# scroll-tech/zkevm-circuits

Measured on NVIDIA H100. Metric: SuperCircuit-shaped k=20 create_proof seconds (halo2 KZG/SHPLONK, Blake2b transcript), lower is better.
Workload: dtype u256 (8x u32 Montgomery limbs, BN254 Fr/Fq)

## Files before the change

### zkevm-circuits_b200/csrc/expr.cu

```cuda
#include <type_traits>
#include "common.cuh"
#include "expr.cuh"

namespace zkb {

struct ExprLaunch {
    const Instr *code;
    uint32_t ncode;
    const Fr *const *cols;
    const Fr *consts;
    Fr *const *outs;
    uint32_t log_n;
    uint32_t out_stride;
    uint32_t out_offset;
};

template <int NREGS, int THREADS, bool SMEM>
struct RegFile {
    uint4 *lo, *hi;
    Fr loc[SMEM ? 1 : NREGS];
    __device__ __forceinline__ RegFile(uint4 *base) : lo(base + threadIdx.x), hi(base + NREGS * THREADS + threadIdx.x) {}
    __device__ __forceinline__ Fr get(uint32_t r) const {
        if (!SMEM) return loc[r];
        const uint4 a = lo[r * THREADS], b = hi[r * THREADS];
        Fr v;
        v.l[0] = a.x; v.l[1] = a.y; v.l[2] = a.z; v.l[3] = a.w;
        v.l[4] = b.x; v.l[5] = b.y; v.l[6] = b.z; v.l[7] = b.w;
        return v;
    }
    __device__ __forceinline__ void set(uint32_t r, const Fr &v) {
        if (!SMEM) { loc[r] = v; return; }
        lo[r * THREADS] = make_uint4(v.l[0], v.l[1], v.l[2], v.l[3]);
        hi[r * THREADS] = make_uint4(v.l[4], v.l[5], v.l[6], v.l[7]);
    }
};

struct FlagLaunch {
    const Instr *code;
    uint32_t ncode;
    const Fr *const *cols;
    const Fr *consts;
    uint32_t *bits;
    uint32_t words;
    uint32_t log_n;
};

template <int NREGS, int THREADS, bool SMEM, class Launch>
__device__ __forceinline__ void run_program(const Launch &L, uint32_t tid) {
    constexpr bool FLAG = std::is_same<Launch, FlagLaunch>::value;
    extern __shared__ uint4 expr_smem[];
    const uint32_t mask = (1u << L.log_n) - 1, row = tid & mask;
    RegFile<NREGS, THREADS, SMEM> regs(expr_smem);
    Fr acc = Fr::zero(), acc2 = Fr::zero();
    uint32_t pc = 0;
    auto col = [&](uint32_t imm) {
        const int32_t rot = (int32_t)(int16_t)(imm >> 16);
        return fp_load(L.cols[imm & 0xffffu] + ((row + (uint32_t)rot) & mask));
    };
    auto cst = [&](uint32_t i) { return fp_load(L.consts + i); };
    auto arg = [&]() { return L.code[++pc].imm; };
    for (; pc < L.ncode; ++pc) {
        const Instr in = L.code[pc];
        Fr x, y;
        switch (in.op) {
        case OP_LOADCOL: regs.set(in.dst, col(in.imm)); continue;
        case OP_LOADCONST: regs.set(in.dst, cst(in.imm)); continue;
        case OP_ADD: x = regs.get(in.a); y = regs.get(in.b); goto add;
        case OP_ADD_RC + FORM_RC: x = regs.get(in.a); y = col(in.imm); goto add;
        case OP_ADD_RC + FORM_CR: x = col(in.imm); y = regs.get(in.a); goto add;
        case OP_ADD_RC + FORM_RK: x = regs.get(in.a); y = cst(in.imm); goto add;
        case OP_ADD_RC + FORM_KR: x = cst(in.imm); y = regs.get(in.a); goto add;
        case OP_ADD_RC + FORM_CC: x = col(in.imm); y = col(arg()); goto add;
        case OP_ADD_RC + FORM_CK: x = col(in.imm); y = cst(arg()); goto add;
        case OP_ADD_RC + FORM_KC: x = cst(in.imm); y = col(arg()); goto add;
        case OP_SUB: x = regs.get(in.a); y = regs.get(in.b); goto sub;
        case OP_SUB_RC + FORM_RC: x = regs.get(in.a); y = col(in.imm); goto sub;
        case OP_SUB_RC + FORM_CR: x = col(in.imm); y = regs.get(in.a); goto sub;
        case OP_SUB_RC + FORM_RK: x = regs.get(in.a); y = cst(in.imm); goto sub;
        case OP_SUB_RC + FORM_KR: x = cst(in.imm); y = regs.get(in.a); goto sub;
        case OP_SUB_RC + FORM_CC: x = col(in.imm); y = col(arg()); goto sub;
        case OP_SUB_RC + FORM_CK: x = col(in.imm); y = cst(arg()); goto sub;
        case OP_SUB_RC + FORM_KC: x = cst(in.imm); y = col(arg()); goto sub;
        case OP_MUL: x = regs.get(in.a); y = regs.get(in.b); goto mul;
        case OP_MUL_RC + FORM_RC: x = regs.get(in.a); y = col(in.imm); goto mul;
        case OP_MUL_RC + FORM_CR: x = col(in.imm); y = regs.get(in.a); goto mul;
        case OP_MUL_RC + FORM_RK: x = regs.get(in.a); y = cst(in.imm); goto mul;
        case OP_MUL_RC + FORM_KR: x = cst(in.imm); y = regs.get(in.a); goto mul;
        case OP_MUL_RC + FORM_CC: x = col(in.imm); y = col(arg()); goto mul;
        case OP_MUL_RC + FORM_CK: x = col(in.imm); y = cst(arg()); goto mul;
        case OP_MUL_RC + FORM_KC: x = cst(in.imm); y = col(arg()); goto mul;
        case OP_NEG: regs.set(in.dst, fp_neg(regs.get(in.a))); continue;
        case OP_FLAG:
            if constexpr (FLAG) {
                const uint32_t b = __ballot_sync(0xffffffffu, tid < (1u << L.log_n) && !regs.get(in.a).is_zero());
                const uint32_t word = tid >> 5;
                if ((threadIdx.x & 31) == 0 && word < L.words) L.bits[(size_t)in.imm * L.words + word] = b;
            }
            continue;
        case OP_HORNER: case OP_HORNER_C:
            if constexpr (!FLAG) acc = fp_add(fp_mul(acc, cst(in.imm)), in.op == OP_HORNER ? regs.get(in.a) : col(arg()));
            continue;
        case OP_HORNER2: case OP_HORNER2_C:
            if constexpr (!FLAG) acc2 = fp_add(fp_mul(acc2, cst(in.imm)), in.op == OP_HORNER2 ? regs.get(in.a) : col(arg()));
            continue;
        case OP_FOLD: case OP_FOLD_C:
            if constexpr (!FLAG) {
                acc = fp_add(fp_mul(acc, cst(in.imm)), fp_mul(in.op == OP_FOLD ? regs.get(in.a) : col(arg()), acc2));
                acc2 = Fr::zero();
            }
            continue;
        case OP_STORE:
            if constexpr (!FLAG) fp_store(L.outs[in.imm] + (size_t)row * L.out_stride + L.out_offset, regs.get(in.a));
            continue;
        case OP_STOREACC:
            if constexpr (!FLAG) fp_store(L.outs[in.imm & 0xffu] + (size_t)row * L.out_stride + L.out_offset, fp_mul(acc, cst(in.imm >> 8)));
            continue;
        case OP_CLEARACC: acc = Fr::zero(); continue;
        default: continue;
        }
    add: regs.set(in.dst, fp_add(x, y)); continue;
    sub: regs.set(in.dst, fp_sub(x, y)); continue;
    mul: regs.set(in.dst, fp_mul(x, y));
    }
}

template <int NREGS, int THREADS, bool SMEM>
__global__ void __launch_bounds__(THREADS) expr_kernel(ExprLaunch L) {
    const uint32_t row = blockIdx.x * blockDim.x + threadIdx.x;
    if (row >= (1u << L.log_n)) return;
    run_program<NREGS, THREADS, SMEM>(L, row);
}

template <int NREGS, int THREADS, bool SMEM>
__global__ void __launch_bounds__(THREADS) expr_flag_kernel(FlagLaunch L) {
    run_program<NREGS, THREADS, SMEM>(L, blockIdx.x * blockDim.x + threadIdx.x);
}

template <class Launch, int NREGS, int THREADS, void (*KERNEL)(Launch)>
static int32_t launch_smem(const Launch &L, uint32_t n, cudaStream_t st) {
    constexpr size_t bytes = (size_t)NREGS * THREADS * 32;
    static bool attr_set[64] = {};
    int dev = 0;
    cudaGetDevice(&dev);
    if (bytes > 48 * 1024 && dev < 64 && !attr_set[dev]) {
        ZKB_CUDA(cudaFuncSetAttribute(KERNEL, cudaFuncAttributeMaxDynamicSharedMemorySize, (int)bytes));
        attr_set[dev] = true;
    }
    KERNEL<<<(n + THREADS - 1) / THREADS, THREADS, bytes, st>>>(L);
    return ZKB_OK;
}

int32_t expr_run_device(zkb_ctx *ctx, const Instr *d_code, uint32_t ncode, int nregs, const Fr *const *d_cols, const Fr *d_consts,
                        Fr *const *d_outs, uint32_t log_n, uint32_t out_stride, uint32_t out_offset, cudaStream_t st) {
    ExprLaunch L{d_code, ncode, d_cols, d_consts, d_outs, log_n, out_stride, out_offset};
    const uint32_t n = 1u << log_n;
    const unsigned blocks = (n + 127) / 128;
    ProfScope ps_(ctx, PROF_EXPR, st);
    if (nregs <= 8) ZKB_TRY((launch_smem<ExprLaunch, 8, 128, expr_kernel<8, 128, true>>(L, n, st)));
    else if (nregs <= 16) ZKB_TRY((launch_smem<ExprLaunch, 16, 128, expr_kernel<16, 128, true>>(L, n, st)));
    else expr_kernel<64, 128, false><<<blocks, 128, 0, st>>>(L);
    ctx->launches++;
    ZKB_CUDA(cudaGetLastError());
    return ZKB_OK;
}

int32_t expr_flag_run_device(zkb_ctx *ctx, const Instr *d_code, uint32_t ncode, int nregs, const Fr *const *d_cols, const Fr *d_consts,
                             uint32_t *bits, uint32_t words, uint32_t log_n, cudaStream_t st) {
    FlagLaunch L{d_code, ncode, d_cols, d_consts, bits, words, log_n};
    const uint32_t n = 1u << log_n;
    if (nregs <= 8) ZKB_TRY((launch_smem<FlagLaunch, 8, 128, expr_flag_kernel<8, 128, true>>(L, n, st)));
    else if (nregs <= 16) ZKB_TRY((launch_smem<FlagLaunch, 16, 128, expr_flag_kernel<16, 128, true>>(L, n, st)));
    else expr_flag_kernel<64, 128, false><<<(n + 127) / 128, 128, 0, st>>>(L);
    ctx->launches++;
    ZKB_CUDA(cudaGetLastError());
    return ZKB_OK;
}

}
```

### zkevm-circuits_b200/csrc/expr.cuh

```cuda
#pragma once
#include <stdint.h>
#include <algorithm>
#include <array>
#include <map>
#include <string>
#include <tuple>
#include <vector>
#include "ff.cuh"

namespace zkb {

enum : uint8_t {
    OP_LOADCOL = 0,
    OP_LOADCONST = 1,
    OP_ADD = 2,
    OP_SUB = 3,
    OP_MUL = 4,
    OP_NEG = 5,
    OP_HORNER = 6,
    OP_STORE = 7,
    OP_STOREACC = 8,
    OP_CLEARACC = 9,
    OP_HORNER2 = 10,
    OP_FOLD = 11,
    OP_FLAG = 12,
    OP_ARG = 13,
    FORM_RC = 0, FORM_CR = 1, FORM_RK = 2, FORM_KR = 3, FORM_CC = 4, FORM_CK = 5, FORM_KC = 6,
    OP_ADD_RC = 16,
    OP_SUB_RC = 24,
    OP_MUL_RC = 32,
    OP_HORNER_C = 40,
    OP_HORNER2_C = 41,
    OP_FOLD_C = 42,
};

struct alignas(8) Instr {
    uint8_t op, dst, a, b;
    uint32_t imm;
};

constexpr int EXPR_MAX_REGS = 64;

struct ENode {
    uint8_t kind;
    uint32_t a, b;
};

class ExprBuilder {
public:
    std::vector<ENode> nodes;
    std::vector<Fr> consts;
    std::vector<uint32_t> degree;

    uint32_t col(uint32_t slot, int32_t rot) { return intern(0, slot, (uint32_t)rot); }
    uint32_t constant(const Fr &v) {
        std::array<uint32_t, 8> key;
        for (int i = 0; i < 8; ++i) key[i] = v.l[i];
        auto it = const_index.find(key);
        uint32_t idx;
        if (it == const_index.end()) {
            idx = (uint32_t)consts.size();
            consts.push_back(v);
            const_index.emplace(key, idx);
        } else idx = it->second;
        return intern(1, idx, 0);
    }
    uint32_t add(uint32_t x, uint32_t y) { return intern(2, x, y); }
    uint32_t sub(uint32_t x, uint32_t y) { return intern(3, x, y); }
    uint32_t mul(uint32_t x, uint32_t y) { return intern(4, x, y); }
    uint32_t neg(uint32_t x) { return intern(5, x, 0); }
    uint32_t const_slot(const Fr &v) {
        uint32_t n = constant(v);
        return nodes[n].a;
    }
    void columns(uint32_t root, std::vector<char> &seen, std::vector<char> &used) const {
        std::vector<uint32_t> stack{root};
        while (!stack.empty()) {
            const uint32_t v = stack.back();
            stack.pop_back();
            if (seen[v]) continue;
            seen[v] = 1;
            const ENode &e = nodes[v];
            if (e.kind == 0) used[e.a] = 1;
            else if (e.kind >= 2) {
                stack.push_back(e.a);
                if (e.kind != 5) stack.push_back(e.b);
            }
        }
    }

private:
    std::map<std::tuple<uint8_t, uint32_t, uint32_t>, uint32_t> index;
    std::map<std::array<uint32_t, 8>, uint32_t> const_index;
    uint32_t intern(uint8_t kind, uint32_t a, uint32_t b) {
        auto key = std::make_tuple(kind, a, b);
        auto it = index.find(key);
        if (it != index.end()) return it->second;
        nodes.push_back(ENode{kind, a, b});
        degree.push_back(kind == 0 ? 1 : kind == 1 ? 0 : kind == 4 ? degree[a] + degree[b] : kind == 5 ? degree[a] : std::max(degree[a], degree[b]));
        index.emplace(key, (uint32_t)nodes.size() - 1);
        return (uint32_t)nodes.size() - 1;
    }
};

class ProgramBuilder {
public:
    explicit ProgramBuilder(ExprBuilder &eb) : eb(eb) {}
    std::vector<Instr> code;
    int max_regs_used = 0;
    std::string error;

    enum RootAction { HORNER, STORE, HORNER2, FOLD, FLAG };
    struct Root { uint32_t node; RootAction action; uint32_t imm; };
    bool scope(const std::vector<Root> &roots);
    void clear_acc() { code.push_back(Instr{OP_CLEARACC, 0, 0, 0, 0}); }
    void store_acc(uint32_t out_slot, uint32_t scale_const_index) {
        code.push_back(Instr{OP_STOREACC, 0, 0, 0, out_slot | (scale_const_index << 8)});
    }

private:
    ExprBuilder &eb;
    void fuse(size_t begin);
};

inline void ProgramBuilder::fuse(size_t begin) {
    auto is_arith = [](uint8_t op) { return op == OP_ADD || op == OP_SUB || op == OP_MUL; };
    auto is_root = [](uint8_t op) { return op == OP_HORNER || op == OP_HORNER2 || op == OP_FOLD; };
    auto is_load = [](uint8_t op) { return op == OP_LOADCOL || op == OP_LOADCONST; };
    auto reads = [&](const Instr &in, int s) {
        if (is_arith(in.op)) return true;
        return s == 0 && (in.op == OP_NEG || is_root(in.op) || in.op == OP_STORE || in.op == OP_FLAG);
    };
    auto writes = [&](const Instr &in) { return is_load(in.op) || is_arith(in.op) || in.op == OP_NEG; };
    const size_t end = code.size();
    std::vector<std::array<int64_t, 2>> src(end - begin, {-1, -1});
    for (size_t i = begin; i < end; ++i) {
        if (!is_load(code[i].op)) continue;
        const uint8_t r = code[i].dst;
        int uses = 0, slot = -1;
        size_t user = 0;
        for (size_t j = i + 1; j < end && uses < 2; ++j) {
            for (int s = 0; s < 2; ++s)
                if (reads(code[j], s) && (s == 0 ? code[j].a : code[j].b) == r) { ++uses; user = j; slot = s; }
            if (writes(code[j]) && code[j].dst == r) break;
        }
        if (uses != 1) continue;
        const uint8_t op = code[user].op;
        if (is_arith(op) || (is_root(op) && code[i].op == OP_LOADCOL)) src[user - begin][slot] = (int64_t)i;
    }
    auto kind = [&](const std::array<int64_t, 2> &s, int k) { return s[k] < 0 ? 'R' : code[s[k]].op == OP_LOADCOL ? 'C' : 'K'; };
    std::vector<bool> fused(end - begin, false);
    for (auto &s : src) {
        if (kind(s, 0) == 'K' && kind(s, 1) == 'K') s[1] = -1;
        for (int k = 0; k < 2; ++k)
            if (s[k] >= 0) fused[s[k] - begin] = true;
    }
    std::vector<Instr> out;
    for (size_t i = begin; i < end; ++i) {
        const Instr in = code[i];
        const auto &s = src[i - begin];
        if (fused[i - begin]) continue;
        if (s[0] < 0 && s[1] < 0) { out.push_back(in); continue; }
        if (is_root(in.op)) {
            const uint8_t op = in.op == OP_HORNER ? OP_HORNER_C : in.op == OP_HORNER2 ? OP_HORNER2_C : OP_FOLD_C;
            out.push_back(Instr{op, 0, 0, 0, in.imm});
            out.push_back(Instr{OP_ARG, 0, 0, 0, code[s[0]].imm});
            continue;
        }
        const char ka = kind(s, 0), kb = kind(s, 1);
        const int form = ka == 'R' ? (kb == 'C' ? FORM_RC : FORM_RK)
                       : kb == 'R' ? (ka == 'C' ? FORM_CR : FORM_KR)
                       : ka == 'C' ? (kb == 'C' ? FORM_CC : FORM_CK) : FORM_KC;
        const uint8_t base = in.op == OP_ADD ? OP_ADD_RC : in.op == OP_SUB ? OP_SUB_RC : OP_MUL_RC;
        const int first = s[0] >= 0 ? 0 : 1;
        const uint8_t reg = ka == 'R' ? in.a : in.b;
        out.push_back(Instr{(uint8_t)(base + form), in.dst, (uint8_t)(form < FORM_CC ? reg : 0), 0, code[s[first]].imm});
        if (form >= FORM_CC) out.push_back(Instr{OP_ARG, 0, 0, 0, code[s[1]].imm});
    }
    code.resize(begin);
    code.insert(code.end(), out.begin(), out.end());
}

inline bool ProgramBuilder::scope(const std::vector<Root> &roots) {
    const size_t begin = code.size();
    std::map<uint32_t, int> refs;
    std::vector<uint32_t> stack;
    std::map<uint32_t, bool> seen;
    for (auto &r : roots) {
        refs[r.node]++;
        if (!seen[r.node]) { seen[r.node] = true; stack.push_back(r.node); }
    }
    while (!stack.empty()) {
        uint32_t n = stack.back();
        stack.pop_back();
        const ENode &e = eb.nodes[n];
        if (e.kind >= 2) {
            uint32_t ch[2] = {e.a, e.b};
            int nch = e.kind == 5 ? 1 : 2;
            for (int i = 0; i < nch; ++i) {
                refs[ch[i]]++;
                if (!seen[ch[i]]) { seen[ch[i]] = true; stack.push_back(ch[i]); }
            }
        }
    }
    std::map<uint32_t, int> reg_of;
    std::vector<int> free_regs;
    for (int i = EXPR_MAX_REGS - 1; i >= 0; --i) free_regs.push_back(i);
    auto alloc = [&]() -> int {
        if (free_regs.empty()) return -1;
        int r = free_regs.back();
        free_regs.pop_back();
        if (r + 1 > max_regs_used) max_regs_used = r + 1;
        return r;
    };
    auto release_use = [&](uint32_t n) {
        if (--refs[n] == 0) {
            free_regs.push_back(reg_of[n]);
            reg_of.erase(n);
        }
    };
    struct Frame { uint32_t node; int state; };
    for (auto &r : roots) {
        if (!reg_of.count(r.node)) {
            std::vector<Frame> st;
            st.push_back({r.node, 0});
            while (!st.empty()) {
                Frame &f = st.back();
                const ENode e = eb.nodes[f.node];
                if (reg_of.count(f.node)) { st.pop_back(); continue; }
                if (e.kind < 2) {
                    int rg = alloc();
                    if (rg < 0) { error = "expression needs more than 64 live registers"; return false; }
                    if (e.kind == 0) code.push_back(Instr{OP_LOADCOL, (uint8_t)rg, 0, 0, (e.a & 0xffffu) | ((uint32_t)(uint16_t)(int16_t)(int32_t)e.b << 16)});
                    else code.push_back(Instr{OP_LOADCONST, (uint8_t)rg, 0, 0, e.a});
                    reg_of[f.node] = rg;
                    st.pop_back();
                    continue;
                }
                const int nch = e.kind == 5 ? 1 : 2;
                if (f.state == 0) {
                    f.state = 1;
                    if (!reg_of.count(e.a)) { st.push_back({e.a, 0}); continue; }
                }
                if (f.state == 1) {
                    f.state = 2;
                    if (nch == 2 && !reg_of.count(e.b)) { st.push_back({e.b, 0}); continue; }
                }
                const int ra = reg_of[e.a];
                const int rb = nch == 2 ? reg_of[e.b] : 0;
                const uint32_t me = f.node;
                release_use(e.a);
                if (nch == 2) release_use(e.b);
                int rg = alloc();
                if (rg < 0) { error = "expression needs more than 64 live registers"; return false; }
                uint8_t op = e.kind == 2 ? OP_ADD : e.kind == 3 ? OP_SUB : e.kind == 4 ? OP_MUL : OP_NEG;
                code.push_back(Instr{op, (uint8_t)rg, (uint8_t)ra, (uint8_t)rb, 0});
                reg_of[me] = rg;
                st.pop_back();
            }
        }
        const int rr = reg_of[r.node];
        if (r.action == HORNER) code.push_back(Instr{OP_HORNER, 0, (uint8_t)rr, 0, r.imm});
        else if (r.action == HORNER2) code.push_back(Instr{OP_HORNER2, 0, (uint8_t)rr, 0, r.imm});
// ... 11 lines not shown
```

### zkevm-circuits_b200/csrc/ff.cuh

```cuda
#pragma once
#include <stdint.h>

#if defined(__CUDACC__)
#define FF_HD __host__ __device__ __forceinline__
#define FF_D __device__ __forceinline__
#else
#define FF_HD inline
#define FF_D inline
#endif

namespace zkb {

struct FrParams {
    static constexpr uint32_t INV = 0xefffffffu;
    FF_HD static constexpr uint32_t P(int i) {
        constexpr uint32_t v[8] = {0xf0000001u, 0x43e1f593u, 0x79b97091u, 0x2833e848u, 0x8181585du, 0xb85045b6u, 0xe131a029u, 0x30644e72u};
        return v[i];
    }
    FF_HD static constexpr uint32_t P2(int i) {
        constexpr uint32_t v[8] = {0xe0000002u, 0x87c3eb27u, 0xf372e122u, 0x5067d090u, 0x0302b0bau, 0x70a08b6du, 0xc2634053u, 0x60c89ce5u};
        return v[i];
    }
    FF_HD static constexpr uint32_t R1(int i) {
        constexpr uint32_t v[8] = {0x4ffffffbu, 0xac96341cu, 0x9f60cd29u, 0x36fc7695u, 0x7879462eu, 0x666ea36fu, 0x9a07df2fu, 0x0e0a77c1u};
// ... 206 lines not shown
    constexpr uint32_t p0 = PR::P(0), p1 = PR::P(1), p2 = PR::P(2), p3 = PR::P(3), p4 = PR::P(4), p5 = PR::P(5), p6 = PR::P(6), p7 = PR::P(7);
#pragma unroll
    for (int i = 0; i < 8; ++i) {
        const uint32_t bi = b.l[i];
        if (i == 0) {
            chain_mad_nc(y0, y1, y2, y3, y4, y5, y6, y7, a.l[1], a.l[3], a.l[5], a.l[7], bi);
        } else {
            uint32_t s = x1;
            uint32_t t0 = x2, t1 = x3, t2 = x4, t3 = x5, t4 = x6, t5 = x7, t6 = x8;
            x0 = y0; x1 = y1; x2 = y2; x3 = y3; x4 = y4; x5 = y5; x6 = y6; x7 = y7; x8 = 0;
            y0 = t0; y1 = t1; y2 = t2; y3 = t3; y4 = t4; y5 = t5; y6 = t6; y7 = 0;
            chain_stray_mad_nc(x0, s, y0, y1, y2, y3, y4, y5, y6, y7, a.l[1], a.l[3], a.l[5], a.l[7], bi);
        }
        chain_mad(x0, x1, x2, x3, x4, x5, x6, x7, x8, a.l[0], a.l[2], a.l[4], a.l[6], bi);
        const uint32_t m = x0 * PR::INV;
        chain_mad(x0, x1, x2, x3, x4, x5, x6, x7, x8, p0, p2, p4, p6, m);
        chain_mad_nc(y0, y1, y2, y3, y4, y5, y6, y7, p1, p3, p5, p7, m);
    }
    asm("add.cc.u32 %0, %8, %16;\n\t"
        "addc.cc.u32 %1, %9, %17;\n\t"
        "addc.cc.u32 %2, %10, %18;\n\t"
        "addc.cc.u32 %3, %11, %19;\n\t"
        "addc.cc.u32 %4, %12, %20;\n\t"
        "addc.cc.u32 %5, %13, %21;\n\t"
        "addc.cc.u32 %6, %14, %22;\n\t"
        "addc.u32 %7, %15, %23;"
        : "=r"(r.l[0]), "=r"(r.l[1]), "=r"(r.l[2]), "=r"(r.l[3]), "=r"(r.l[4]), "=r"(r.l[5]), "=r"(r.l[6]), "=r"(r.l[7])
        : "r"(x1), "r"(x2), "r"(x3), "r"(x4), "r"(x5), "r"(x6), "r"(x7), "r"(x8),
          "r"(y0), "r"(y1), "r"(y2), "r"(y3), "r"(y4), "r"(y5), "r"(y6), "r"(y7));
    if (!REDUCE) return r;
    Fp<PR> t;
    uint32_t borrow;
    asm("sub.cc.u32 %0, %9, %17;\n\t"
        "subc.cc.u32 %1, %10, %18;\n\t"
        "subc.cc.u32 %2, %11, %19;\n\t"
        "subc.cc.u32 %3, %12, %20;\n\t"
        "subc.cc.u32 %4, %13, %21;\n\t"
        "subc.cc.u32 %5, %14, %22;\n\t"
        "subc.cc.u32 %6, %15, %23;\n\t"
        "subc.cc.u32 %7, %16, %24;\n\t"
        "subc.u32 %8, 0, 0;"
        : "=r"(t.l[0]), "=r"(t.l[1]), "=r"(t.l[2]), "=r"(t.l[3]), "=r"(t.l[4]), "=r"(t.l[5]), "=r"(t.l[6]), "=r"(t.l[7]), "=r"(borrow)
        : "r"(r.l[0]), "r"(r.l[1]), "r"(r.l[2]), "r"(r.l[3]), "r"(r.l[4]), "r"(r.l[5]), "r"(r.l[6]), "r"(r.l[7]),
          "r"(p0), "r"(p1), "r"(p2), "r"(p3), "r"(p4), "r"(p5), "r"(p6), "r"(p7));
#pragma unroll
    for (int i = 0; i < 8; ++i) r.l[i] = borrow ? r.l[i] : t.l[i];
#else
    uint64_t A[4], B[4], P64[4], t[6] = {0, 0, 0, 0, 0, 0};
    for (int i = 0; i < 4; ++i) {
        A[i] = (uint64_t)a.l[2 * i] | ((uint64_t)a.l[2 * i + 1] << 32);
        B[i] = (uint64_t)b.l[2 * i] | ((uint64_t)b.l[2 * i + 1] << 32);
        P64[i] = (uint64_t)PR::P(2 * i) | ((uint64_t)PR::P(2 * i + 1) << 32);
    }
    uint64_t inv64 = PR::INV;
    inv64 = inv64 * (2 + P64[0] * inv64);
    typedef unsigned __int128 u128;
    for (int i = 0; i < 4; ++i) {
        u128 c = 0;
        for (int j = 0; j < 4; ++j) { c += (u128)A[j] * B[i] + t[j]; t[j] = (uint64_t)c; c >>= 64; }
        c += t[4]; t[4] = (uint64_t)c; t[5] = (uint64_t)(c >> 64);
        const uint64_t m = t[0] * inv64;
        c = (u128)m * P64[0] + t[0]; c >>= 64;
        for (int j = 1; j < 4; ++j) { c += (u128)m * P64[j] + t[j]; t[j - 1] = (uint64_t)c; c >>= 64; }
        c += t[4]; t[3] = (uint64_t)c; t[4] = t[5] + (uint64_t)(c >> 64);
    }
    uint64_t u[4];
    u128 br = 0;
    for (int i = 0; i < 4; ++i) { u128 d = (u128)t[i] - P64[i] - (uint64_t)br; u[i] = (uint64_t)d; br = (d >> 64) & 1; }
    const bool ge = t[4] != 0 || br == 0;
    for (int i = 0; i < 4; ++i) {
        const uint64_t v = ge ? u[i] : t[i];
        r.l[2 * i] = (uint32_t)v;
        r.l[2 * i + 1] = (uint32_t)(v >> 32);
    }
#endif
    return r;
}

template <class PR>
FF_HD Fp<PR> fp_mul(const Fp<PR> &a, const Fp<PR> &b) { return fp_mul_t<PR, true>(a, b); }
template <class PR>
FF_HD Fp<PR> fp_mul_lazy(const Fp<PR> &a, const Fp<PR> &b) { return fp_mul_t<PR, false>(a, b); }

template <class PR>
FF_HD Fp<PR> fp_sqr(const Fp<PR> &a) {
    return fp_mul(a, a);
}

#if defined(__CUDACC__)
template <class PR>
__device__ __forceinline__ Fp<PR> fp_add_lazy(const Fp<PR> &a, const Fp<PR> &b) {
    Fp<PR> r, t;
    asm("add.cc.u32 %0, %8, %16;\n\t"
        "addc.cc.u32 %1, %9, %17;\n\t"
        "addc.cc.u32 %2, %10, %18;\n\t"
        "addc.cc.u32 %3, %11, %19;\n\t"
        "addc.cc.u32 %4, %12, %20;\n\t"
        "addc.cc.u32 %5, %13, %21;\n\t"
        "addc.cc.u32 %6, %14, %22;\n\t"
        "addc.u32 %7, %15, %23;"
        : "=r"(r.l[0]), "=r"(r.l[1]), "=r"(r.l[2]), "=r"(r.l[3]), "=r"(r.l[4]), "=r"(r.l[5]), "=r"(r.l[6]), "=r"(r.l[7])
        : "r"(a.l[0]), "r"(a.l[1]), "r"(a.l[2]), "r"(a.l[3]), "r"(a.l[4]), "r"(a.l[5]), "r"(a.l[6]), "r"(a.l[7]),
          "r"(b.l[0]), "r"(b.l[1]), "r"(b.l[2]), "r"(b.l[3]), "r"(b.l[4]), "r"(b.l[5]), "r"(b.l[6]), "r"(b.l[7]));
    uint32_t borrow;
    asm("sub.cc.u32 %0, %9, %17;\n\t"
        "subc.cc.u32 %1, %10, %18;\n\t"
        "subc.cc.u32 %2, %11, %19;\n\t"
        "subc.cc.u32 %3, %12, %20;\n\t"
        "subc.cc.u32 %4, %13, %21;\n\t"
        "subc.cc.u32 %5, %14, %22;\n\t"
        "subc.cc.u32 %6, %15, %23;\n\t"
        "subc.cc.u32 %7, %16, %24;\n\t"
        "subc.u32 %8, 0, 0;"
        : "=r"(t.l[0]), "=r"(t.l[1]), "=r"(t.l[2]), "=r"(t.l[3]), "=r"(t.l[4]), "=r"(t.l[5]), "=r"(t.l[6]), "=r"(t.l[7]), "=r"(borrow)
        : "r"(r.l[0]), "r"(r.l[1]), "r"(r.l[2]), "r"(r.l[3]), "r"(r.l[4]), "r"(r.l[5]), "r"(r.l[6]), "r"(r.l[7]),
          "r"(PR::P2(0)), "r"(PR::P2(1)), "r"(PR::P2(2)), "r"(PR::P2(3)), "r"(PR::P2(4)), "r"(PR::P2(5)), "r"(PR::P2(6)), "r"(PR::P2(7)));
#pragma unroll
    for (int i = 0; i < 8; ++i) r.l[i] = borrow ? r.l[i] : t.l[i];
    return r;
}
template <class PR>
__device__ __forceinline__ Fp<PR> fp_sub_lazy(const Fp<PR> &a, const Fp<PR> &b) {
    Fp<PR> r;
    asm("sub.cc.u32 %0, %8, %16;\n\t"
        "subc.cc.u32 %1, %9, %17;\n\t"
        "subc.cc.u32 %2, %10, %18;\n\t"
        "subc.cc.u32 %3, %11, %19;\n\t"
        "subc.cc.u32 %4, %12, %20;\n\t"
        "subc.cc.u32 %5, %13, %21;\n\t"
        "subc.cc.u32 %6, %14, %22;\n\t"
        "subc.u32 %7, %15, %23;"
        : "=r"(r.l[0]), "=r"(r.l[1]), "=r"(r.l[2]), "=r"(r.l[3]), "=r"(r.l[4]), "=r"(r.l[5]), "=r"(r.l[6]), "=r"(r.l[7])
        : "r"(a.l[0]), "r"(a.l[1]), "r"(a.l[2]), "r"(a.l[3]), "r"(a.l[4]), "r"(a.l[5]), "r"(a.l[6]), "r"(a.l[7]),
          "r"(b.l[0]), "r"(b.l[1]), "r"(b.l[2]), "r"(b.l[3]), "r"(b.l[4]), "r"(b.l[5]), "r"(b.l[6]), "r"(b.l[7]));
    asm("add.cc.u32 %0, %0, %8;\n\t"
        "addc.cc.u32 %1, %1, %9;\n\t"
        "addc.cc.u32 %2, %2, %10;\n\t"
        "addc.cc.u32 %3, %3, %11;\n\t"
        "addc.cc.u32 %4, %4, %12;\n\t"
        "addc.cc.u32 %5, %5, %13;\n\t"
        "addc.cc.u32 %6, %6, %14;\n\t"
        "addc.u32 %7, %7, %15;"
        : "+r"(r.l[0]), "+r"(r.l[1]), "+r"(r.l[2]), "+r"(r.l[3]), "+r"(r.l[4]), "+r"(r.l[5]), "+r"(r.l[6]), "+r"(r.l[7])
        : "r"(PR::P2(0)), "r"(PR::P2(1)), "r"(PR::P2(2)), "r"(PR::P2(3)), "r"(PR::P2(4)), "r"(PR::P2(5)), "r"(PR::P2(6)), "r"(PR::P2(7)));
    return r;
}
template <class PR, bool TWO>
__device__ __forceinline__ Fp<PR> fp_cond_sub(const Fp<PR> &x) {
    Fp<PR> t, r;
    uint32_t borrow;
    asm("sub.cc.u32 %0, %9, %17;\n\t"
        "subc.cc.u32 %1, %10, %18;\n\t"
        "subc.cc.u32 %2, %11, %19;\n\t"
        "subc.cc.u32 %3, %12, %20;\n\t"
        "subc.cc.u32 %4, %13, %21;\n\t"
        "subc.cc.u32 %5, %14, %22;\n\t"
        "subc.cc.u32 %6, %15, %23;\n\t"
        "subc.cc.u32 %7, %16, %24;\n\t"
        "subc.u32 %8, 0, 0;"
        : "=r"(t.l[0]), "=r"(t.l[1]), "=r"(t.l[2]), "=r"(t.l[3]), "=r"(t.l[4]), "=r"(t.l[5]), "=r"(t.l[6]), "=r"(t.l[7]), "=r"(borrow)
        : "r"(x.l[0]), "r"(x.l[1]), "r"(x.l[2]), "r"(x.l[3]), "r"(x.l[4]), "r"(x.l[5]), "r"(x.l[6]), "r"(x.l[7]),
          "r"(TWO ? PR::P2(0) : PR::P(0)), "r"(TWO ? PR::P2(1) : PR::P(1)), "r"(TWO ? PR::P2(2) : PR::P(2)), "r"(TWO ? PR::P2(3) : PR::P(3)),
          "r"(TWO ? PR::P2(4) : PR::P(4)), "r"(TWO ? PR::P2(5) : PR::P(5)), "r"(TWO ? PR::P2(6) : PR::P(6)), "r"(TWO ? PR::P2(7) : PR::P(7)));
#pragma unroll
    for (int i = 0; i < 8; ++i) r.l[i] = borrow ? x.l[i] : t.l[i];
    return r;
}
#endif

// ... 90 lines not shown
```

### zkevm-circuits_b200/csrc/g1.cuh

```cuda
#pragma once
#include "ff.cuh"

namespace zkb {

struct alignas(32) G1Affine {
    Fq x, y;
    FF_HD bool is_identity() const { return x.is_zero() && y.is_zero(); }
};

struct alignas(32) G1Xyzz {
    Fq x, y, zz, zzz;
    FF_HD bool is_identity() const { return zz.is_zero(); }
    FF_HD static G1Xyzz identity() {
        G1Xyzz r;
        r.x = Fq::zero(); r.y = Fq::zero(); r.zz = Fq::zero(); r.zzz = Fq::zero();
        return r;
    }
    FF_HD static G1Xyzz from_affine(const G1Affine &p) {
        if (p.is_identity()) return identity();
        G1Xyzz r;
        r.x = p.x; r.y = p.y; r.zz = Fq::one(); r.zzz = Fq::one();
        return r;
    }
};

FF_HD G1Xyzz g1_dbl_affine(const G1Affine &p) {
    if (p.is_identity()) return G1Xyzz::identity();
    G1Xyzz r;
    Fq u = fp_dbl(p.y);
    Fq v = fp_sqr(u);
    Fq w = fp_mul(u, v);
    Fq s = fp_mul(p.x, v);
    Fq xx = fp_sqr(p.x);
    Fq m = fp_add(fp_dbl(xx), xx);
    r.x = fp_sub(fp_sqr(m), fp_dbl(s));
    r.y = fp_sub(fp_mul(m, fp_sub(s, r.x)), fp_mul(w, p.y));
    r.zz = v;
    r.zzz = w;
    return r;
}

FF_HD G1Xyzz g1_dbl(const G1Xyzz &p) {
    if (p.is_identity()) return p;
    G1Xyzz r;
    Fq u = fp_dbl(p.y);
    Fq v = fp_sqr(u);
    Fq w = fp_mul(u, v);
    Fq s = fp_mul(p.x, v);
    Fq xx = fp_sqr(p.x);
    Fq m = fp_add(fp_dbl(xx), xx);
    r.x = fp_sub(fp_sqr(m), fp_dbl(s));
    r.y = fp_sub(fp_mul(m, fp_sub(s, r.x)), fp_mul(w, p.y));
    r.zz = fp_mul(v, p.zz);
    r.zzz = fp_mul(w, p.zzz);
    return r;
}

FF_HD void g1_add_mixed(G1Xyzz &acc, const G1Affine &q) {
    if (q.is_identity()) return;
    if (acc.is_identity()) { acc = G1Xyzz::from_affine(q); return; }
    Fq u2 = fp_mul(q.x, acc.zz);
    Fq s2 = fp_mul(q.y, acc.zzz);
    Fq p = fp_sub(u2, acc.x);
    Fq r = fp_sub(s2, acc.y);
    if (p.is_zero()) {
        if (r.is_zero()) acc = g1_dbl_affine(q);
        else acc = G1Xyzz::identity();
        return;
    }
    Fq pp = fp_sqr(p);
    Fq ppp = fp_mul(p, pp);
    Fq qq = fp_mul(acc.x, pp);
    Fq x3 = fp_sub(fp_sub(fp_sqr(r), ppp), fp_dbl(qq));
    Fq y3 = fp_sub(fp_mul(r, fp_sub(qq, x3)), fp_mul(acc.y, ppp));
    acc.x = x3;
    acc.y = y3;
    acc.zz = fp_mul(acc.zz, pp);
    acc.zzz = fp_mul(acc.zzz, ppp);
}

FF_HD void g1_add(G1Xyzz &acc, const G1Xyzz &q) {
    if (q.is_identity()) return;
    if (acc.is_identity()) { acc = q; return; }
    Fq u1 = fp_mul(acc.x, q.zz);
    Fq u2 = fp_mul(q.x, acc.zz);
    Fq s1 = fp_mul(acc.y, q.zzz);
    Fq s2 = fp_mul(q.y, acc.zzz);
    Fq p = fp_sub(u2, u1);
    Fq r = fp_sub(s2, s1);
    if (p.is_zero()) {
        if (r.is_zero()) acc = g1_dbl(acc);
        else acc = G1Xyzz::identity();
        return;
    }
    Fq pp = fp_sqr(p);
    Fq ppp = fp_mul(p, pp);
    Fq qq = fp_mul(u1, pp);
    Fq x3 = fp_sub(fp_sub(fp_sqr(r), ppp), fp_dbl(qq));
    Fq y3 = fp_sub(fp_mul(r, fp_sub(qq, x3)), fp_mul(s1, ppp));
    acc.x = x3;
    acc.y = y3;
    acc.zz = fp_mul(fp_mul(acc.zz, q.zz), pp);
    acc.zzz = fp_mul(fp_mul(acc.zzz, q.zzz), ppp);
}

FF_HD G1Affine g1_neg(const G1Affine &p) {
    G1Affine r;
    r.x = p.x;
    r.y = p.is_identity() ? p.y : fp_neg(p.y);
    return r;
}

FF_HD G1Affine g1_to_affine(const G1Xyzz &p) {
    G1Affine r;
    if (p.is_identity()) { r.x = Fq::zero(); r.y = Fq::zero(); return r; }
    Fq t = fp_inv(fp_mul(p.zz, p.zzz));
    Fq zz_inv = fp_mul(t, p.zzz);
    Fq zzz_inv = fp_mul(t, p.zz);
    r.x = fp_mul(p.x, zz_inv);
    r.y = fp_mul(p.y, zzz_inv);
    return r;
}

inline void g1_compress(const G1Affine &p, uint8_t out[32]) {
    if (p.is_identity()) { for (int i = 0; i < 32; ++i) out[i] = 0; return; }
    Fq x = fp_to_canonical(p.x), y = fp_to_canonical(p.y);
    for (int i = 0; i < 8; ++i) {
        out[4 * i + 0] = (uint8_t)(x.l[i]);
        out[4 * i + 1] = (uint8_t)(x.l[i] >> 8);
        out[4 * i + 2] = (uint8_t)(x.l[i] >> 16);
        out[4 * i + 3] = (uint8_t)(x.l[i] >> 24);
    }
    out[31] |= (uint8_t)((y.l[0] & 1u) << 6);
}

#if defined(__CUDACC__)
FF_D G1Affine g1_load_affine(const G1Affine *p) {
    G1Affine r;
    r.x = fp_load(&p->x);
    r.y = fp_load(&p->y);
    return r;
}
FF_D void g1_store_affine(G1Affine *p, const G1Affine &v) {
    fp_store(&p->x, v.x);
    fp_store(&p->y, v.y);
}
FF_D G1Xyzz g1_load_xyzz(const G1Xyzz *p) {
    G1Xyzz r;
    r.x = fp_load(&p->x); r.y = fp_load(&p->y); r.zz = fp_load(&p->zz); r.zzz = fp_load(&p->zzz);
    return r;
}
FF_D void g1_store_xyzz(G1Xyzz *p, const G1Xyzz &v) {
    fp_store(&p->x, v.x); fp_store(&p->y, v.y); fp_store(&p->zz, v.zz); fp_store(&p->zzz, v.zzz);
}
#endif

}
```

Before: 1.666.

## Add fused mul-add-mul Montgomery kernel, dedicated squaring, and Horner product fusion

Adds a sum-of-products Montgomery routine that folds a*b + c*d into a single reduction, and uses it for the y-coordinate in the G1 doubling and addition formulas through a negate-then-add variant. Replaces the generic squaring with a wide schoolbook square that computes each cross term once and then reduces. The expression bytecode builder gains a pass that merges a single-use MUL feeding a HORNER step into new HORNER_M opcodes, and the interpreter evaluates these and FOLD through the fused routine. The aim is fewer Montgomery reductions in MSM and quotient evaluation, at the cost of more complex carry chains, higher register pressure, and a riskier peephole pass in the code generator.

```diff
diff --git a/zkevm-circuits_b200/csrc/expr.cu b/zkevm-circuits_b200/csrc/expr.cu
--- a/zkevm-circuits_b200/csrc/expr.cu
+++ b/zkevm-circuits_b200/csrc/expr.cu
@@ -61,7 +61,7 @@
     auto arg = [&]() { return L.code[++pc].imm; };
     for (; pc < L.ncode; ++pc) {
         const Instr in = L.code[pc];
-        Fr x, y;
+        Fr x, y, z, w;
         switch (in.op) {
         case OP_LOADCOL: regs.set(in.dst, col(in.imm)); continue;
         case OP_LOADCONST: regs.set(in.dst, cst(in.imm)); continue;
@@ -104,11 +104,16 @@
             if constexpr (!FLAG) acc2 = fp_add(fp_mul(acc2, cst(in.imm)), in.op == OP_HORNER2 ? regs.get(in.a) : col(arg()));
             continue;
         case OP_FOLD: case OP_FOLD_C:
-            if constexpr (!FLAG) {
-                acc = fp_add(fp_mul(acc, cst(in.imm)), fp_mul(in.op == OP_FOLD ? regs.get(in.a) : col(arg()), acc2));
-                acc2 = Fr::zero();
-            }
-            continue;
+            if constexpr (FLAG) continue;
+            else { x = acc; y = cst(in.imm); z = in.op == OP_FOLD ? regs.get(in.a) : col(arg()); w = acc2; goto mac; }
+        case OP_HORNER_M: case OP_HORNER2_M:
+            if constexpr (FLAG) continue;
+            else if constexpr (!SMEM) {
+                const Fr t = fp_mul(regs.get(in.a), regs.get(in.b));
+                if (in.op == OP_HORNER_M) acc = fp_add(fp_mul(acc, cst(in.imm)), t);
+                else acc2 = fp_add(fp_mul(acc2, cst(in.imm)), t);
+                continue;
+            } else { x = in.op == OP_HORNER_M ? acc : acc2; y = cst(in.imm); z = regs.get(in.a); w = regs.get(in.b); goto mac; }
         case OP_STORE:
             if constexpr (!FLAG) fp_store(L.outs[in.imm] + (size_t)row * L.out_stride + L.out_offset, regs.get(in.a));
             continue;
@@ -120,7 +125,15 @@
         }
     add: regs.set(in.dst, fp_add(x, y)); continue;
     sub: regs.set(in.dst, fp_sub(x, y)); continue;
-    mul: regs.set(in.dst, fp_mul(x, y));
+    mul: regs.set(in.dst, fp_mul(x, y)); continue;
+    mac: {
+        const Fr r = fp_mul_add_mul(x, y, z, w);
+        if (in.op == OP_HORNER2_M) acc2 = r;
+        else {
+            acc = r;
+            if (in.op != OP_HORNER_M) acc2 = Fr::zero();
+        }
+    }
     }
 }
 
diff --git a/zkevm-circuits_b200/csrc/expr.cuh b/zkevm-circuits_b200/csrc/expr.cuh
--- a/zkevm-circuits_b200/csrc/expr.cuh
+++ b/zkevm-circuits_b200/csrc/expr.cuh
@@ -32,6 +32,8 @@
     OP_HORNER_C = 40,
     OP_HORNER2_C = 41,
     OP_FOLD_C = 42,
+    OP_HORNER_M = 43,
+    OP_HORNER2_M = 44,
 };
 
 struct alignas(8) Instr {
@@ -121,6 +123,7 @@
 private:
     ExprBuilder &eb;
     void fuse(size_t begin);
+    static void merge_products(std::vector<Instr> &code);
 };
 
 inline void ProgramBuilder::fuse(size_t begin) {
@@ -177,8 +180,58 @@
         out.push_back(Instr{(uint8_t)(base + form), in.dst, (uint8_t)(form < FORM_CC ? reg : 0), 0, code[s[first]].imm});
         if (form >= FORM_CC) out.push_back(Instr{OP_ARG, 0, 0, 0, code[s[1]].imm});
     }
+    merge_products(out);
     code.resize(begin);
     code.insert(code.end(), out.begin(), out.end());
+}
+
+inline void ProgramBuilder::merge_products(std::vector<Instr> &code) {
+    const size_t n = code.size();
+    auto reg_reads = [](const Instr &in, int s) {
+        const uint8_t op = in.op;
+        if (op == OP_ADD || op == OP_SUB || op == OP_MUL) return true;
+        if (s != 0) return false;
+        if (op == OP_NEG || op == OP_HORNER || op == OP_HORNER2 || op == OP_FOLD || op == OP_STORE || op == OP_FLAG) return true;
+        return op >= OP_ADD_RC && op < OP_MUL_RC + 8 && (op & 7) < FORM_CC;
+    };
+    auto reg_writes = [](const Instr &in) {
+        const uint8_t op = in.op;
+        return op == OP_LOADCOL || op == OP_LOADCONST || op == OP_ADD || op == OP_SUB || op == OP_MUL || op == OP_NEG ||
+               (op >= OP_ADD_RC && op < OP_MUL_RC + 8);
+    };
+    std::vector<int64_t> reader(n, -1);
+    for (size_t i = 0; i < n; ++i) {
+        const Instr &m = code[i];
+        if (m.op != OP_MUL) continue;
+        int uses = 0;
+        size_t user = 0;
+        for (size_t j = i + 1; j < n && uses < 2; ++j) {
+            for (int s = 0; s < 2; ++s)
+                if (reg_reads(code[j], s) && (s == 0 ? code[j].a : code[j].b) == m.dst) { ++uses; user = j; }
+            if (reg_writes(code[j]) && code[j].dst == m.dst) break;
+        }
+        if (uses != 1) continue;
+        bool intact = true;
+        for (size_t j = i + 1; j < user; ++j)
+            if (reg_writes(code[j]) && (code[j].dst == m.a || code[j].dst == m.b)) intact = false;
+        if (intact) reader[i] = (int64_t)user;
+    }
+    std::vector<int64_t> prod(n, -1);
+    for (size_t i = 0; i < n; ++i)
+        if (reader[i] >= 0 && (code[reader[i]].op == OP_HORNER || code[reader[i]].op == OP_HORNER2)) prod[reader[i]] = (int64_t)i;
+    std::vector<bool> merged(n, false);
+    std::vector<Instr> out;
+    for (size_t j = 0; j < n; ++j) {
+        Instr in = code[j];
+        if (prod[j] >= 0) {
+            in = Instr{(uint8_t)(in.op == OP_HORNER ? OP_HORNER_M : OP_HORNER2_M), 0, code[prod[j]].a, code[prod[j]].b, in.imm};
+            merged[prod[j]] = true;
+        }
+        out.push_back(in);
+    }
+    code.clear();
+    for (size_t j = 0; j < n; ++j)
+        if (!merged[j]) code.push_back(out[j]);
 }
 
 inline bool ProgramBuilder::scope(const std::vector<Root> &roots) {
diff --git a/zkevm-circuits_b200/csrc/ff.cuh b/zkevm-circuits_b200/csrc/ff.cuh
--- a/zkevm-circuits_b200/csrc/ff.cuh
+++ b/zkevm-circuits_b200/csrc/ff.cuh
@@ -312,9 +312,296 @@
 template <class PR>
 FF_HD Fp<PR> fp_mul_lazy(const Fp<PR> &a, const Fp<PR> &b) { return fp_mul_t<PR, false>(a, b); }
 
+#if defined(__CUDA_ARCH__)
+namespace detail {
+template <int K>
+FF_D void mad_row(uint32_t *c, const uint32_t *e, uint32_t b) {
+    if constexpr (K == 4) {
+        chain_mad(c[0], c[1], c[2], c[3], c[4], c[5], c[6], c[7], c[8], e[0], e[1], e[2], e[3], b);
+    } else if constexpr (K == 3) {
+        asm("mad.lo.cc.u32 %0, %7, %10, %0;\n\t"
+            "madc.hi.cc.u32 %1, %7, %10, %1;\n\t"
+            "madc.lo.cc.u32 %2, %8, %10, %2;\n\t"
+            "madc.hi.cc.u32 %3, %8, %10, %3;\n\t"
+            "madc.lo.cc.u32 %4, %9, %10, %4;\n\t"
+            "madc.hi.cc.u32 %5, %9, %10, %5;\n\t"
+            "addc.u32 %6, %6, 0;"
+            : "+r"(c[0]), "+r"(c[1]), "+r"(c[2]), "+r"(c[3]), "+r"(c[4]), "+r"(c[5]), "+r"(c[6])
+            : "r"(e[0]), "r"(e[1]), "r"(e[2]), "r"(b));
+    } else if constexpr (K == 2) {
+        asm("mad.lo.cc.u32 %0, %5, %7, %0;\n\t"
+            "madc.hi.cc.u32 %1, %5, %7, %1;\n\t"
+            "madc.lo.cc.u32 %2, %6, %7, %2;\n\t"
+            "madc.hi.cc.u32 %3, %6, %7, %3;\n\t"
+            "addc.u32 %4, %4, 0;"
+            : "+r"(c[0]), "+r"(c[1]), "+r"(c[2]), "+r"(c[3]), "+r"(c[4])
+            : "r"(e[0]), "r"(e[1]), "r"(b));
+    } else {
+        static_assert(K == 1, "rows of 1 to 4 products");
+        asm("mad.lo.cc.u32 %0, %3, %4, %0;\n\t"
+            "madc.hi.cc.u32 %1, %3, %4, %1;\n\t"
+            "addc.u32 %2, %2, 0;"
+            : "+r"(c[0]), "+r"(c[1]), "+r"(c[2])
+            : "r"(e[0]), "r"(b));
+    }
+}
+
+struct Wide {
+    uint32_t E[17], O[17];
+    FF_D Wide() {
+#pragma unroll
+        for (int i = 0; i < 17; ++i) E[i] = O[i] = 0;
+    }
+    FF_D void sum(uint32_t T[16]) const {
+        T[0] = E[0];
+        asm("add.cc.u32 %0, %15, %30;\n\t"
+            "addc.cc.u32 %1, %16, %31;\n\t"
+            "addc.cc.u32 %2, %17, %32;\n\t"
+            "addc.cc.u32 %3, %18, %33;\n\t"
+            "addc.cc.u32 %4, %19, %34;\n\t"
+            "addc.cc.u32 %5, %20, %35;\n\t"
+            "addc.cc.u32 %6, %21, %36;\n\t"
+            "addc.cc.u32 %7, %22, %37;\n\t"
+            "addc.cc.u32 %8, %23, %38;\n\t"
+            "addc.cc.u32 %9, %24, %39;\n\t"
+            "addc.cc.u32 %10, %25, %40;\n\t"
+            "addc.cc.u32 %11, %26, %41;\n\t"
+            "addc.cc.u32 %12, %27, %42;\n\t"
+            "addc.cc.u32 %13, %28, %43;\n\t"
+            "addc.u32 %14, %29, %44;"
+            : "=r"(T[1]), "=r"(T[2]), "=r"(T[3]), "=r"(T[4]), "=r"(T[5]), "=r"(T[6]), "=r"(T[7]), "=r"(T[8]), "=r"(T[9]), "=r"(T[10]),
+              "=r"(T[11]), "=r"(T[12]), "=r"(T[13]), "=r"(T[14]), "=r"(T[15])
+            : "r"(E[1]), "r"(E[2]), "r"(E[3]), "r"(E[4]), "r"(E[5]), "r"(E[6]), "r"(E[7]), "r"(E[8]), "r"(E[9]), "r"(E[10]), "r"(E[11]),
+              "r"(E[12]), "r"(E[13]), "r"(E[14]), "r"(E[15]),
+              "r"(O[1]), "r"(O[2]), "r"(O[3]), "r"(O[4]), "r"(O[5]), "r"(O[6]), "r"(O[7]), "r"(O[8]), "r"(O[9]), "r"(O[10]), "r"(O[11]),
+              "r"(O[12]), "r"(O[13]), "r"(O[14]), "r"(O[15]));
+    }
+};
+
+FF_D void wide_sqr(const uint32_t *a, uint32_t T[16]) {
+    Wide w;
+#pragma unroll
+    for (int i = 0; i < 7; ++i) {
+        uint32_t od[4], ev[4];
+        int no = 0, ne = 0;
+#pragma unroll
+        for (int j = i + 1; j < 8; j += 2) od[no++] = a[j];
+#pragma unroll
+        for (int j = i + 2; j < 8; j += 2) ev[ne++] = a[j];
+        switch (no) {
+        case 4: mad_row<4>(w.O + 2 * i + 1, od, a[i]); break;
+        case 3: mad_row<3>(w.O + 2 * i + 1, od, a[i]); break;
+        case 2: mad_row<2>(w.O + 2 * i + 1, od, a[i]); break;
+        default: mad_row<1>(w.O + 2 * i + 1, od, a[i]); break;
+        }
+        switch (ne) {
+        case 3: mad_row<3>(w.E + 2 * i + 2, ev, a[i]); break;
+        case 2: mad_row<2>(w.E + 2 * i + 2, ev, a[i]); break;
+        case 1: mad_row<1>(w.E + 2 * i + 2, ev, a[i]); break;
+        default: break;
+        }
+    }
+    w.sum(T);
+    asm("add.cc.u32 %0, %0, %0;\n\t"
+        "addc.cc.u32 %1, %1, %1;\n\t"
+        "addc.cc.u32 %2, %2, %2;\n\t"
+        "addc.cc.u32 %3, %3, %3;\n\t"
+        "addc.cc.u32 %4, %4, %4;\n\t"
+        "addc.cc.u32 %5, %5, %5;\n\t"
+        "addc.cc.u32 %6, %6, %6;\n\t"
+        "addc.cc.u32 %7, %7, %7;\n\t"
+        "addc.cc.u32 %8, %8, %8;\n\t"
+        "addc.cc.u32 %9, %9, %9;\n\t"
+        "addc.cc.u32 %10, %10, %10;\n\t"
+        "addc.cc.u32 %11, %11, %11;\n\t"
+        "addc.cc.u32 %12, %12, %12;\n\t"
+        "addc.cc.u32 %13, %13, %13;\n\t"
+        "addc.cc.u32 %14, %14, %14;\n\t"
+        "addc.u32 %15, %15, %15;\n\t"
+        "mad.lo.cc.u32 %0, %16, %16, %0;\n\t"
+        "madc.hi.cc.u32 %1, %16, %16, %1;\n\t"
+        "madc.lo.cc.u32 %2, %17, %17, %2;\n\t"
+        "madc.hi.cc.u32 %3, %17, %17, %3;\n\t"
+        "madc.lo.cc.u32 %4, %18, %18, %4;\n\t"
+        "madc.hi.cc.u32 %5, %18, %18, %5;\n\t"
+        "madc.lo.cc.u32 %6, %19, %19, %6;\n\t"
+        "madc.hi.cc.u32 %7, %19, %19, %7;\n\t"
+        "madc.lo.cc.u32 %8, %20, %20, %8;\n\t"
+        "madc.hi.cc.u32 %9, %20, %20, %9;\n\t"
+        "madc.lo.cc.u32 %10, %21, %21, %10;\n\t"
+        "madc.hi.cc.u32 %11, %21, %21, %11;\n\t"
+        "madc.lo.cc.u32 %12, %22, %22, %12;\n\t"
+        "madc.hi.cc.u32 %13, %22, %22, %13;\n\t"
+        "madc.lo.cc.u32 %14, %23, %23, %14;\n\t"
+        "madc.hi.u32 %15, %23, %23, %15;"
+        : "+r"(T[0]), "+r"(T[1]), "+r"(T[2]), "+r"(T[3]), "+r"(T[4]), "+r"(T[5]), "+r"(T[6]), "+r"(T[7]), "+r"(T[8]), "+r"(T[9]),
+          "+r"(T[10]), "+r"(T[11]), "+r"(T[12]), "+r"(T[13]), "+r"(T[14]), "+r"(T[15])
+        : "r"(a[0]), "r"(a[1]), "r"(a[2]), "r"(a[3]), "r"(a[4]), "r"(a[5]), "r"(a[6]), "r"(a[7]));
+}
+
+template <class PR>
+FF_D Fp<PR> redc(const uint32_t T[16]) {
+    constexpr uint32_t p0 = PR::P(0), p1 = PR::P(1), p2 = PR::P(2), p3 = PR::P(3), p4 = PR::P(4), p5 = PR::P(5), p6 = PR::P(6), p7 = PR::P(7);
+    uint32_t x0 = T[0], x1 = T[1], x2 = T[2], x3 = T[3], x4 = T[4], x5 = T[5], x6 = T[6], x7 = T[7], x8 = 0;
+    uint32_t y0 = 0, y1 = 0, y2 = 0, y3 = 0, y4 = 0, y5 = 0, y6 = 0, y7 = 0;
+#pragma unroll
+    for (int i = 0; i < 8; ++i) {
+        uint32_t m;
+        if (i == 0) {
+            m = x0 * PR::INV;
+            chain_mad_nc(y0, y1, y2, y3, y4, y5, y6, y7, p1, p3, p5, p7, m);
+        } else {
+            const uint32_t s = x1;
+            const uint32_t t0 = x2, t1 = x3, t2 = x4, t3 = x5, t4 = x6, t5 = x7, t6 = x8;
+            x0 = y0; x1 = y1; x2 = y2; x3 = y3; x4 = y4; x5 = y5; x6 = y6; x7 = y7; x8 = 0;
+            y0 = t0; y1 = t1; y2 = t2; y3 = t3; y4 = t4; y5 = t5; y6 = t6; y7 = 0;
+            asm("add.cc.u32 %0, %0, %10;\n\t"
+                "mul.lo.u32 %9, %0, %11;\n\t"
+                "madc.lo.cc.u32 %1, %12, %9, %1;\n\t"
+                "madc.hi.cc.u32 %2, %12, %9, %2;\n\t"
+                "madc.lo.cc.u32 %3, %13, %9, %3;\n\t"
+                "madc.hi.cc.u32 %4, %13, %9, %4;\n\t"
+                "madc.lo.cc.u32 %5, %14, %9, %5;\n\t"
+                "madc.hi.cc.u32 %6, %14, %9, %6;\n\t"
+                "madc.lo.cc.u32 %7, %15, %9, %7;\n\t"
+                "madc.hi.u32 %8, %15, %9, %8;"
+                : "+r"(x0), "+r"(y0), "+r"(y1), "+r"(y2), "+r"(y3), "+r"(y4), "+r"(y5), "+r"(y6), "+r"(y7), "=r"(m)
+                : "r"(s), "r"(PR::INV), "r"(p1), "r"(p3), "r"(p5), "r"(p7));
+        }
+        chain_mad(x0, x1, x2, x3, x4, x5, x6, x7, x8, p0, p2, p4, p6, m);
+    }
+    Fp<PR> r;
+    asm("add.cc.u32 %0, %8, %16;\n\t"
+        "addc.cc.u32 %1, %9, %17;\n\t"
+        "addc.cc.u32 %2, %10, %18;\n\t"
+        "addc.cc.u32 %3, %11, %19;\n\t"
+        "addc.cc.u32 %4, %12, %20;\n\t"
+        "addc.cc.u32 %5, %13, %21;\n\t"
+        "addc.cc.u32 %6, %14, %22;\n\t"
+        "addc.u32 %7, %15, %23;"
+        : "=r"(r.l[0]), "=r"(r.l[1]), "=r"(r.l[2]), "=r"(r.l[3]), "=r"(r.l[4]), "=r"(r.l[5]), "=r"(r.l[6]), "=r"(r.l[7])
+        : "r"(x1), "r"(x2), "r"(x3), "r"(x4), "r"(x5), "r"(x6), "r"(x7), "r"(x8),
+          "r"(y0), "r"(y1), "r"(y2), "r"(y3), "r"(y4), "r"(y5), "r"(y6), "r"(y7));
+    asm("add.cc.u32 %0, %0, %8;\n\t"
+        "addc.cc.u32 %1, %1, %9;\n\t"
+        "addc.cc.u32 %2, %2, %10;\n\t"
+        "addc.cc.u32 %3, %3, %11;\n\t"
+        "addc.cc.u32 %4, %4, %12;\n\t"
+        "addc.cc.u32 %5, %5, %13;\n\t"
+        "addc.cc.u32 %6, %6, %14;\n\t"
+        "addc.u32 %7, %7, %15;"
+        : "+r"(r.l[0]), "+r"(r.l[1]), "+r"(r.l[2]), "+r"(r.l[3]), "+r"(r.l[4]), "+r"(r.l[5]), "+r"(r.l[6]), "+r"(r.l[7])
+        : "r"(T[8]), "r"(T[9]), "r"(T[10]), "r"(T[11]), "r"(T[12]), "r"(T[13]), "r"(T[14]), "r"(T[15]));
+    Fp<PR> t;
+    uint32_t borrow;
+    asm("sub.cc.u32 %0, %9, %17;\n\t"
+        "subc.cc.u32 %1, %10, %18;\n\t"
+        "subc.cc.u32 %2, %11, %19;\n\t"
+        "subc.cc.u32 %3, %12, %20;\n\t"
+        "subc.cc.u32 %4, %13, %21;\n\t"
+        "subc.cc.u32 %5, %14, %22;\n\t"
+        "subc.cc.u32 %6, %15, %23;\n\t"
+        "subc.cc.u32 %7, %16, %24;\n\t"
+        "subc.u32 %8, 0, 0;"
+        : "=r"(t.l[0]), "=r"(t.l[1]), "=r"(t.l[2]), "=r"(t.l[3]), "=r"(t.l[4]), "=r"(t.l[5]), "=r"(t.l[6]), "=r"(t.l[7]), "=r"(borrow)
+        : "r"(r.l[0]), "r"(r.l[1]), "r"(r.l[2]), "r"(r.l[3]), "r"(r.l[4]), "r"(r.l[5]), "r"(r.l[6]), "r"(r.l[7]),
+          "r"(p0), "r"(p1), "r"(p2), "r"(p3), "r"(p4), "r"(p5), "r"(p6), "r"(p7));
+#pragma unroll
+    for (int i = 0; i < 8; ++i) r.l[i] = borrow ? r.l[i] : t.l[i];
+    return r;
+}
+}
+#endif
+
 template <class PR>
 FF_HD Fp<PR> fp_sqr(const Fp<PR> &a) {
+#if defined(__CUDA_ARCH__)
+    uint32_t T[16];
+    detail::wide_sqr(a.l, T);
+    return detail::redc<PR>(T);
+#else
     return fp_mul(a, a);
+#endif
+}
+
+template <class PR>
+FF_HD Fp<PR> fp_mul_add_mul(const Fp<PR> &a, const Fp<PR> &b, const Fp<PR> &c, const Fp<PR> &d) {
+#if defined(__CUDA_ARCH__)
+    using namespace detail;
+    uint32_t x0 = 0, x1 = 0, x2 = 0, x3 = 0, x4 = 0, x5 = 0, x6 = 0, x7 = 0, x8 = 0;
+    uint32_t y0 = 0, y1 = 0, y2 = 0, y3 = 0, y4 = 0, y5 = 0, y6 = 0, y7 = 0;
+    constexpr uint32_t p0 = PR::P(0), p1 = PR::P(1), p2 = PR::P(2), p3 = PR::P(3), p4 = PR::P(4), p5 = PR::P(5), p6 = PR::P(6), p7 = PR::P(7);
+#pragma unroll
+    for (int i = 0; i < 8; ++i) {
+        const uint32_t bi = b.l[i], di = d.l[i];
+        if (i == 0) {
+            chain_mad_nc(y0, y1, y2, y3, y4, y5, y6, y7, a.l[1], a.l[3], a.l[5], a.l[7], bi);
+        } else {
+            uint32_t s = x1;
+            uint32_t t0 = x2, t1 = x3, t2 = x4, t3 = x5, t4 = x6, t5 = x7, t6 = x8;
+            x0 = y0; x1 = y1; x2 = y2; x3 = y3; x4 = y4; x5 = y5; x6 = y6; x7 = y7; x8 = 0;
+            y0 = t0; y1 = t1; y2 = t2; y3 = t3; y4 = t4; y5 = t5; y6 = t6; y7 = 0;
+            chain_stray_mad_nc(x0, s, y0, y1, y2, y3, y4, y5, y6, y7, a.l[1], a.l[3], a.l[5], a.l[7], bi);
+        }
+        chain_mad_nc(y0, y1, y2, y3, y4, y5, y6, y7, c.l[1], c.l[3], c.l[5], c.l[7], di);
+        chain_mad(x0, x1, x2, x3, x4, x5, x6, x7, x8, a.l[0], a.l[2], a.l[4], a.l[6], bi);
+        chain_mad(x0, x1, x2, x3, x4, x5, x6, x7, x8, c.l[0], c.l[2], c.l[4], c.l[6], di);
+        const uint32_t m = x0 * PR::INV;
+        chain_mad(x0, x1, x2, x3, x4, x5, x6, x7, x8, p0, p2, p4, p6, m);
+        chain_mad_nc(y0, y1, y2, y3, y4, y5, y6, y7, p1, p3, p5, p7, m);
+    }
+    Fp<PR> r, t;
+    asm("add.cc.u32 %0, %8, %16;\n\t"
+        "addc.cc.u32 %1, %9, %17;\n\t"
+        "addc.cc.u32 %2, %10, %18;\n\t"
+        "addc.cc.u32 %3, %11, %19;\n\t"
+        "addc.cc.u32 %4, %12, %20;\n\t"
+        "addc.cc.u32 %5, %13, %21;\n\t"
+        "addc.cc.u32 %6, %14, %22;\n\t"
+        "addc.u32 %7, %15, %23;"
+        : "=r"(r.l[0]), "=r"(r.l[1]), "=r"(r.l[2]), "=r"(r.l[3]), "=r"(r.l[4]), "=r"(r.l[5]), "=r"(r.l[6]), "=r"(r.l[7])
+        : "r"(x1), "r"(x2), "r"(x3), "r"(x4), "r"(x5), "r"(x6), "r"(x7), "r"(x8),
+          "r"(y0), "r"(y1), "r"(y2), "r"(y3), "r"(y4), "r"(y5), "r"(y6), "r"(y7));
+    uint32_t borrow;
+    asm("sub.cc.u32 %0, %9, %17;\n\t"
+        "subc.cc.u32 %1, %10, %18;\n\t"
+        "subc.cc.u32 %2, %11, %19;\n\t"
+        "subc.cc.u32 %3, %12, %20;\n\t"
+        "subc.cc.u32 %4, %13, %21;\n\t"
+        "subc.cc.u32 %5, %14, %22;\n\t"
+        "subc.cc.u32 %6, %15, %23;\n\t"
+        "subc.cc.u32 %7, %16, %24;\n\t"
+        "subc.u32 %8, 0, 0;"
+        : "=r"(t.l[0]), "=r"(t.l[1]), "=r"(t.l[2]), "=r"(t.l[3]), "=r"(t.l[4]), "=r"(t.l[5]), "=r"(t.l[6]), "=r"(t.l[7]), "=r"(borrow)
+        : "r"(r.l[0]), "r"(r.l[1]), "r"(r.l[2]), "r"(r.l[3]), "r"(r.l[4]), "r"(r.l[5]), "r"(r.l[6]), "r"(r.l[7]),
+          "r"(p0), "r"(p1), "r"(p2), "r"(p3), "r"(p4), "r"(p5), "r"(p6), "r"(p7));
+#pragma unroll
+    for (int i = 0; i < 8; ++i) r.l[i] = borrow ? r.l[i] : t.l[i];
+    return r;
+#else
+    return fp_add(fp_mul(a, b), fp_mul(c, d));
+#endif
+}
+
+template <class PR>
+FF_HD Fp<PR> fp_mul_sub_mul(const Fp<PR> &a, const Fp<PR> &b, const Fp<PR> &c, const Fp<PR> &d) {
+#if defined(__CUDA_ARCH__)
+    Fp<PR> nc;
+    asm("sub.cc.u32 %0, %8, %16;\n\t"
+        "subc.cc.u32 %1, %9, %17;\n\t"
+        "subc.cc.u32 %2, %10, %18;\n\t"
+        "subc.cc.u32 %3, %11, %19;\n\t"
+        "subc.cc.u32 %4, %12, %20;\n\t"
+        "subc.cc.u32 %5, %13, %21;\n\t"
+        "subc.cc.u32 %6, %14, %22;\n\t"
+        "subc.u32 %7, %15, %23;"
+        : "=r"(nc.l[0]), "=r"(nc.l[1]), "=r"(nc.l[2]), "=r"(nc.l[3]), "=r"(nc.l[4]), "=r"(nc.l[5]), "=r"(nc.l[6]), "=r"(nc.l[7])
+        : "r"(PR::P(0)), "r"(PR::P(1)), "r"(PR::P(2)), "r"(PR::P(3)), "r"(PR::P(4)), "r"(PR::P(5)), "r"(PR::P(6)), "r"(PR::P(7)),
+          "r"(c.l[0]), "r"(c.l[1]), "r"(c.l[2]), "r"(c.l[3]), "r"(c.l[4]), "r"(c.l[5]), "r"(c.l[6]), "r"(c.l[7]));
+    return fp_mul_add_mul(a, b, nc, d);
+#else
+    return fp_sub(fp_mul(a, b), fp_mul(c, d));
+#endif
 }
 
 #if defined(__CUDACC__)
diff --git a/zkevm-circuits_b200/csrc/g1.cuh b/zkevm-circuits_b200/csrc/g1.cuh
--- a/zkevm-circuits_b200/csrc/g1.cuh
+++ b/zkevm-circuits_b200/csrc/g1.cuh
@@ -34,7 +34,7 @@
     Fq xx = fp_sqr(p.x);
     Fq m = fp_add(fp_dbl(xx), xx);
     r.x = fp_sub(fp_sqr(m), fp_dbl(s));
-    r.y = fp_sub(fp_mul(m, fp_sub(s, r.x)), fp_mul(w, p.y));
+    r.y = fp_mul_sub_mul(m, fp_sub(s, r.x), w, p.y);
     r.zz = v;
     r.zzz = w;
     return r;
@@ -50,7 +50,7 @@
     Fq xx = fp_sqr(p.x);
     Fq m = fp_add(fp_dbl(xx), xx);
     r.x = fp_sub(fp_sqr(m), fp_dbl(s));
-    r.y = fp_sub(fp_mul(m, fp_sub(s, r.x)), fp_mul(w, p.y));
+    r.y = fp_mul_sub_mul(m, fp_sub(s, r.x), w, p.y);
     r.zz = fp_mul(v, p.zz);
     r.zzz = fp_mul(w, p.zzz);
     return r;
@@ -72,7 +72,7 @@
     Fq ppp = fp_mul(p, pp);
     Fq qq = fp_mul(acc.x, pp);
     Fq x3 = fp_sub(fp_sub(fp_sqr(r), ppp), fp_dbl(qq));
-    Fq y3 = fp_sub(fp_mul(r, fp_sub(qq, x3)), fp_mul(acc.y, ppp));
+    Fq y3 = fp_mul_sub_mul(r, fp_sub(qq, x3), acc.y, ppp);
     acc.x = x3;
     acc.y = y3;
     acc.zz = fp_mul(acc.zz, pp);
@@ -97,7 +97,7 @@
     Fq ppp = fp_mul(p, pp);
     Fq qq = fp_mul(u1, pp);
     Fq x3 = fp_sub(fp_sub(fp_sqr(r), ppp), fp_dbl(qq));
-    Fq y3 = fp_sub(fp_mul(r, fp_sub(qq, x3)), fp_mul(s1, ppp));
+    Fq y3 = fp_mul_sub_mul(r, fp_sub(qq, x3), s1, ppp);
     acc.x = x3;
     acc.y = y3;
     acc.zz = fp_mul(fp_mul(acc.zz, q.zz), pp);
```

Measured after the change: 1.614 (median of 6 runs). 1.03x faster.
